# reazon-research/ReazonSpeech

Measured on NVIDIA H100. Metric: RTFx (audio-s/wall-s) FastConformer-RNNT 619M, higher is better.
Workload: dtype bf16

## Files before the change

reazonspeech_b200/csrc/common.cuh:

```cuda
#pragma once
#include <cuda_bf16.h>
#include <cuda_fp16.h>
#include <cuda_runtime.h>
#include <stdint.h>

#include <atomic>

namespace rs {

struct DeviceOnce {
  std::atomic<unsigned long long> done{0};
  bool pending() const { int d = 0; cudaGetDevice(&d); return ((done.load(std::memory_order_acquire) >> (d & 63)) & 1ull) == 0; }
  void set() { int d = 0; cudaGetDevice(&d); done.fetch_or(1ull << (d & 63), std::memory_order_release); }
};

constexpr int kWarp = 32;

__device__ __forceinline__ uint32_t smem_u32(const void* p) {
  return static_cast<uint32_t>(__cvta_generic_to_shared(p));
}
__device__ __forceinline__ int lane_id() { return threadIdx.x & 31; }
__device__ __forceinline__ int warp_id_uniform() { return __shfl_sync(0xffffffffu, threadIdx.x >> 5, 0); }

__device__ __forceinline__ float warp_sum(float v) {
#pragma unroll
  for (int o = 16; o > 0; o >>= 1) v += __shfl_xor_sync(0xffffffffu, v, o);
  return v;
}
__device__ __forceinline__ float warp_max(float v) {
#pragma unroll
  for (int o = 16; o > 0; o >>= 1) v = fmaxf(v, __shfl_xor_sync(0xffffffffu, v, o));
  return v;
}

__device__ __forceinline__ uint32_t pack_bf16x2(float lo, float hi) {
  __nv_bfloat162 t = __floats2bfloat162_rn(lo, hi);
  return *reinterpret_cast<uint32_t*>(&t);
}
__device__ __forceinline__ uint32_t pack_f16x2(float lo, float hi) {
  __half2 t = __floats2half2_rn(lo, hi);
  return *reinterpret_cast<uint32_t*>(&t);
}
__device__ __forceinline__ float2 unpack_bf16x2(uint32_t v) {
  __nv_bfloat162 t = *reinterpret_cast<__nv_bfloat162*>(&v);
  return __bfloat1622float2(t);
}
__device__ __forceinline__ float bf16_lo(uint32_t v) { return __uint_as_float(v << 16); }
__device__ __forceinline__ float bf16_hi(uint32_t v) { return __uint_as_float(v & 0xffff0000u); }

__device__ __forceinline__ void split2(float2 x, uint32_t& hi, uint32_t& lo) {
  constexpr float kMax = 65504.f;
  const __half2 h = __floats2half2_rn(fminf(fmaxf(x.x, -kMax), kMax), fminf(fmaxf(x.y, -kMax), kMax));
  const float2 hf = __half22float2(h);
  const __half2 l = __floats2half2_rn(fminf(fmaxf(x.x - hf.x, -kMax), kMax), fminf(fmaxf(x.y - hf.y, -kMax), kMax));
  hi = *reinterpret_cast<const uint32_t*>(&h);
  lo = *reinterpret_cast<const uint32_t*>(&l);
}

__device__ __forceinline__ uint32_t bf16x2_to_f16x2(uint32_t v) { return pack_f16x2(bf16_lo(v), bf16_hi(v)); }
__device__ __forceinline__ uint4 bf16x8_to_f16x8(uint4 v) {
  return make_uint4(bf16x2_to_f16x2(v.x), bf16x2_to_f16x2(v.y), bf16x2_to_f16x2(v.z), bf16x2_to_f16x2(v.w));
}

__device__ __forceinline__ float sigmoidf_fast(float x) {
  float e, r;
  asm("ex2.approx.ftz.f32 %0, %1;" : "=f"(e) : "f"(x * -1.4426950408889634f));
  asm("rcp.approx.ftz.f32 %0, %1;" : "=f"(r) : "f"(1.0f + e));
  return r;
}
__device__ __forceinline__ float sigmoidf_accurate(float x) { return 1.0f / (1.0f + expf(-x)); }
__device__ __forceinline__ float swishf_fast(float x) { return x * sigmoidf_fast(x); }

__device__ __forceinline__ void mbar_init(uint32_t bar, uint32_t count) {
  asm volatile("mbarrier.init.shared::cta.b64 [%0], %1;" ::"r"(bar), "r"(count));
}
__device__ __forceinline__ void fence_barrier_init() {
  asm volatile("fence.mbarrier_init.release.cluster;" ::: "memory");
}
__device__ __forceinline__ void fence_proxy_async() {
  asm volatile("fence.proxy.async.shared::cta;" ::: "memory");
}
__device__ __forceinline__ void mbar_arrive(uint32_t bar) {
  asm volatile("mbarrier.arrive.shared::cta.b64 _, [%0];" ::"r"(bar) : "memory");
}
__device__ __forceinline__ void mbar_arrive_expect_tx(uint32_t bar, uint32_t bytes) {
  asm volatile("mbarrier.arrive.expect_tx.shared::cta.b64 _, [%0], %1;" ::"r"(bar), "r"(bytes) : "memory");
}
__device__ __forceinline__ bool mbar_try_wait(uint32_t bar, uint32_t parity) {
  uint32_t ok;
  asm volatile(
      "{\n\t.reg .pred p;\n\t"
      "mbarrier.try_wait.parity.shared::cta.b64 p, [%1], %2;\n\t"
      "selp.u32 %0, 1, 0, p;\n\t}"
      : "=r"(ok)
      : "r"(bar), "r"(parity)
      : "memory");
  return ok != 0;
}
__device__ __forceinline__ void mbar_wait(uint32_t bar, uint32_t parity) {
  while (!mbar_try_wait(bar, parity)) {
  }
}

__device__ __forceinline__ void tma_prefetch_desc(const void* desc) {
  asm volatile("prefetch.tensormap [%0];" ::"l"(desc) : "memory");
}
__device__ __forceinline__ void tma_load_2d(uint32_t smem_dst, const void* desc, int c0, int c1, uint32_t bar) {
  asm volatile(
      "cp.async.bulk.tensor.2d.shared::cluster.global.tile.mbarrier::complete_tx::bytes [%0], [%1, {%3, %4}], [%2];"
      ::"r"(smem_dst), "l"(desc), "r"(bar), "r"(c0), "r"(c1)
      : "memory");
}

__device__ __forceinline__ void tma_store_2d(const void* desc, uint32_t smem_src, int c0, int c1) {
  asm volatile("cp.async.bulk.tensor.2d.global.shared::cta.bulk_group [%0, {%2, %3}], [%1];"
               ::"l"(desc), "r"(smem_src), "r"(c0), "r"(c1) : "memory");
}
__device__ __forceinline__ void tma_reduce_add_2d(const void* desc, uint32_t smem_src, int c0, int c1) {
  asm volatile("cp.reduce.async.bulk.tensor.2d.global.shared::cta.add.tile.bulk_group [%0, {%2, %3}], [%1];"
               ::"l"(desc), "r"(smem_src), "r"(c0), "r"(c1) : "memory");
}
__device__ __forceinline__ void bulk_commit() { asm volatile("cp.async.bulk.commit_group;" ::: "memory"); }
template <int N>
__device__ __forceinline__ void bulk_wait_read() { asm volatile("cp.async.bulk.wait_group.read %0;" ::"n"(N) : "memory"); }
template <int N>
__device__ __forceinline__ void bulk_wait() { asm volatile("cp.async.bulk.wait_group %0;" ::"n"(N) : "memory"); }

__device__ __forceinline__ void cp_async16(void* smem, const void* gmem) {
  asm volatile("cp.async.cg.shared.global [%0], [%1], 16;" ::"r"(smem_u32(smem)), "l"(gmem) : "memory");
}
__device__ __forceinline__ void cp_async_wait_all() { asm volatile("cp.async.wait_all;" ::: "memory"); }

__device__ __forceinline__ void stmatrix_x4(uint32_t addr, uint32_t r0, uint32_t r1, uint32_t r2, uint32_t r3) {
  asm volatile("stmatrix.sync.aligned.m8n8.x4.shared.b16 [%0], {%1, %2, %3, %4};"
               ::"r"(addr), "r"(r0), "r"(r1), "r"(r2), "r"(r3) : "memory");
}
__device__ __forceinline__ void stmatrix_x4_trans(uint32_t addr, uint32_t r0, uint32_t r1, uint32_t r2, uint32_t r3) {
  asm volatile("stmatrix.sync.aligned.m8n8.x4.trans.shared.b16 [%0], {%1, %2, %3, %4};"
               ::"r"(addr), "r"(r0), "r"(r1), "r"(r2), "r"(r3) : "memory");
}

template <int N>
__device__ __forceinline__ void setmaxnreg_dec() { asm volatile("setmaxnreg.dec.sync.aligned.u32 %0;" ::"n"(N)); }
template <int N>
__device__ __forceinline__ void setmaxnreg_inc() { asm volatile("setmaxnreg.inc.sync.aligned.u32 %0;" ::"n"(N)); }

__device__ __forceinline__ void wgmma_fence() { asm volatile("wgmma.fence.sync.aligned;" ::: "memory"); }
__device__ __forceinline__ void wgmma_commit() { asm volatile("wgmma.commit_group.sync.aligned;" ::: "memory"); }
template <int N>
__device__ __forceinline__ void wgmma_wait() { asm volatile("wgmma.wait_group.sync.aligned %0;" ::"n"(N) : "memory"); }
__device__ __forceinline__ void named_bar_sync(int id, int threads) { asm volatile("bar.sync %0, %1;" ::"r"(id), "r"(threads) : "memory"); }

__device__ __forceinline__ uint64_t wgmma_desc_k_sw128(uint32_t smem_addr) {
  uint64_t d = 0;
  d |= static_cast<uint64_t>((smem_addr & 0x3ffffu) >> 4);
  d |= static_cast<uint64_t>(1) << 16;
  d |= static_cast<uint64_t>(1024 >> 4) << 32;
  d |= static_cast<uint64_t>(1) << 62;
  return d;
}

__device__ __forceinline__ void wgmma_bf16_ss_n32(float (&d)[16], uint64_t desc_a, uint64_t desc_b, uint32_t accumulate) {
  asm volatile(
      "{\n\t.reg .pred p;\n\t"
      "setp.ne.b32 p, %18, 0;\n\t"
      "wgmma.mma_async.sync.aligned.m64n32k16.f32.bf16.bf16 "
      "{%0, %1, %2, %3, %4, %5, %6, %7, %8, %9, %10, %11, %12, %13, %14, %15}, %16, %17, p, 1, 1, 0, 0;\n\t}"
      :
        "+f"(d[0]), "+f"(d[1]), "+f"(d[2]), "+f"(d[3]), "+f"(d[4]), "+f"(d[5]), "+f"(d[6]), "+f"(d[7]),
        "+f"(d[8]), "+f"(d[9]), "+f"(d[10]), "+f"(d[11]), "+f"(d[12]), "+f"(d[13]), "+f"(d[14]), "+f"(d[15])
      : "l"(desc_a), "l"(desc_b), "r"(accumulate));
}

__device__ __forceinline__ void wgmma_bf16_ss_n64(float (&d)[32], uint64_t desc_a, uint64_t desc_b, uint32_t accumulate) {
  asm volatile(
      "{\n\t.reg .pred p;\n\t"
      "setp.ne.b32 p, %34, 0;\n\t"
      "wgmma.mma_async.sync.aligned.m64n64k16.f32.bf16.bf16 "
      "{%0, %1, %2, %3, %4, %5, %6, %7, %8, %9, %10, %11, %12, %13, %14, %15, %16, %17, %18, %19, %20, %21, %22, %23, %24, %25, %26, %27, %28, %29, %30, %31}, %32, %33, p, 1, 1, 0, 0;\n\t}"
      :
        "+f"(d[0]), "+f"(d[1]), "+f"(d[2]), "+f"(d[3]), "+f"(d[4]), "+f"(d[5]), "+f"(d[6]), "+f"(d[7]),
        "+f"(d[8]), "+f"(d[9]), "+f"(d[10]), "+f"(d[11]), "+f"(d[12]), "+f"(d[13]), "+f"(d[14]), "+f"(d[15]),
        "+f"(d[16]), "+f"(d[17]), "+f"(d[18]), "+f"(d[19]), "+f"(d[20]), "+f"(d[21]), "+f"(d[22]), "+f"(d[23]),
        "+f"(d[24]), "+f"(d[25]), "+f"(d[26]), "+f"(d[27]), "+f"(d[28]), "+f"(d[29]), "+f"(d[30]), "+f"(d[31])
      : "l"(desc_a), "l"(desc_b), "r"(accumulate));
}

__device__ __forceinline__ void wgmma_bf16_ss_n128(float (&d)[64], uint64_t desc_a, uint64_t desc_b, uint32_t accumulate) {
  asm volatile(
      "{\n\t.reg .pred p;\n\t"
      "setp.ne.b32 p, %66, 0;\n\t"
      "wgmma.mma_async.sync.aligned.m64n128k16.f32.bf16.bf16 "
      "{%0, %1, %2, %3, %4, %5, %6, %7, %8, %9, %10, %11, %12, %13, %14, %15, %16, %17, %18, %19, %20, %21, %22, %23, %24, %25, %26, %27, %28, %29, %30, %31, %32, %33, %34, %35, %36, %37, %38, %39, %40, %41, %42, %43, %44, %45, %46, %47, %48, %49, %50, %51, %52, %53, %54, %55, %56, %57, %58, %59, %60, %61, %62, %63}, %64, %65, p, 1, 1, 0, 0;\n\t}"
      :
        "+f"(d[0]), "+f"(d[1]), "+f"(d[2]), "+f"(d[3]), "+f"(d[4]), "+f"(d[5]), "+f"(d[6]), "+f"(d[7]),
        "+f"(d[8]), "+f"(d[9]), "+f"(d[10]), "+f"(d[11]), "+f"(d[12]), "+f"(d[13]), "+f"(d[14]), "+f"(d[15]),
        "+f"(d[16]), "+f"(d[17]), "+f"(d[18]), "+f"(d[19]), "+f"(d[20]), "+f"(d[21]), "+f"(d[22]), "+f"(d[23]),
        "+f"(d[24]), "+f"(d[25]), "+f"(d[26]), "+f"(d[27]), "+f"(d[28]), "+f"(d[29]), "+f"(d[30]), "+f"(d[31]),
        "+f"(d[32]), "+f"(d[33]), "+f"(d[34]), "+f"(d[35]), "+f"(d[36]), "+f"(d[37]), "+f"(d[38]), "+f"(d[39]),
        "+f"(d[40]), "+f"(d[41]), "+f"(d[42]), "+f"(d[43]), "+f"(d[44]), "+f"(d[45]), "+f"(d[46]), "+f"(d[47]),
        "+f"(d[48]), "+f"(d[49]), "+f"(d[50]), "+f"(d[51]), "+f"(d[52]), "+f"(d[53]), "+f"(d[54]), "+f"(d[55]),
        "+f"(d[56]), "+f"(d[57]), "+f"(d[58]), "+f"(d[59]), "+f"(d[60]), "+f"(d[61]), "+f"(d[62]), "+f"(d[63])
      : "l"(desc_a), "l"(desc_b), "r"(accumulate));
}

__device__ __forceinline__ void wgmma_bf16_ss_n256(float (&d)[128], uint64_t desc_a, uint64_t desc_b, uint32_t accumulate) {
  asm volatile(
      "{\n\t.reg .pred p;\n\t"
      "setp.ne.b32 p, %130, 0;\n\t"
      "wgmma.mma_async.sync.aligned.m64n256k16.f32.bf16.bf16 "
      "{%0, %1, %2, %3, %4, %5, %6, %7, %8, %9, %10, %11, %12, %13, %14, %15, %16, %17, %18, %19, %20, %21, %22, %23, %24, %25, %26, %27, %28, %29, %30, %31, "
      "%32, %33, %34, %35, %36, %37, %38, %39, %40, %41, %42, %43, %44, %45, %46, %47, %48, %49, %50, %51, %52, %53, %54, %55, %56, %57, %58, %59, %60, %61, %62, %63, "
      "%64, %65, %66, %67, %68, %69, %70, %71, %72, %73, %74, %75, %76, %77, %78, %79, %80, %81, %82, %83, %84, %85, %86, %87, %88, %89, %90, %91, %92, %93, %94, %95, "
      "%96, %97, %98, %99, %100, %101, %102, %103, %104, %105, %106, %107, %108, %109, %110, %111, %112, %113, %114, %115, %116, %117, %118, %119, %120, %121, %122, %123, %124, %125, %126, %127}, "
      "%128, %129, p, 1, 1, 0, 0;\n\t}"
      :
        "+f"(d[0]), "+f"(d[1]), "+f"(d[2]), "+f"(d[3]), "+f"(d[4]), "+f"(d[5]), "+f"(d[6]), "+f"(d[7]),
        "+f"(d[8]), "+f"(d[9]), "+f"(d[10]), "+f"(d[11]), "+f"(d[12]), "+f"(d[13]), "+f"(d[14]), "+f"(d[15]),
        "+f"(d[16]), "+f"(d[17]), "+f"(d[18]), "+f"(d[19]), "+f"(d[20]), "+f"(d[21]), "+f"(d[22]), "+f"(d[23]),
        "+f"(d[24]), "+f"(d[25]), "+f"(d[26]), "+f"(d[27]), "+f"(d[28]), "+f"(d[29]), "+f"(d[30]), "+f"(d[31]),
        "+f"(d[32]), "+f"(d[33]), "+f"(d[34]), "+f"(d[35]), "+f"(d[36]), "+f"(d[37]), "+f"(d[38]), "+f"(d[39]),
        "+f"(d[40]), "+f"(d[41]), "+f"(d[42]), "+f"(d[43]), "+f"(d[44]), "+f"(d[45]), "+f"(d[46]), "+f"(d[47]),
        "+f"(d[48]), "+f"(d[49]), "+f"(d[50]), "+f"(d[51]), "+f"(d[52]), "+f"(d[53]), "+f"(d[54]), "+f"(d[55]),
        "+f"(d[56]), "+f"(d[57]), "+f"(d[58]), "+f"(d[59]), "+f"(d[60]), "+f"(d[61]), "+f"(d[62]), "+f"(d[63]),
        "+f"(d[64]), "+f"(d[65]), "+f"(d[66]), "+f"(d[67]), "+f"(d[68]), "+f"(d[69]), "+f"(d[70]), "+f"(d[71]),
        "+f"(d[72]), "+f"(d[73]), "+f"(d[74]), "+f"(d[75]), "+f"(d[76]), "+f"(d[77]), "+f"(d[78]), "+f"(d[79]),
        "+f"(d[80]), "+f"(d[81]), "+f"(d[82]), "+f"(d[83]), "+f"(d[84]), "+f"(d[85]), "+f"(d[86]), "+f"(d[87]),
        "+f"(d[88]), "+f"(d[89]), "+f"(d[90]), "+f"(d[91]), "+f"(d[92]), "+f"(d[93]), "+f"(d[94]), "+f"(d[95]),
        "+f"(d[96]), "+f"(d[97]), "+f"(d[98]), "+f"(d[99]), "+f"(d[100]), "+f"(d[101]), "+f"(d[102]), "+f"(d[103]),
        "+f"(d[104]), "+f"(d[105]), "+f"(d[106]), "+f"(d[107]), "+f"(d[108]), "+f"(d[109]), "+f"(d[110]), "+f"(d[111]),
        "+f"(d[112]), "+f"(d[113]), "+f"(d[114]), "+f"(d[115]), "+f"(d[116]), "+f"(d[117]), "+f"(d[118]), "+f"(d[119]),
        "+f"(d[120]), "+f"(d[121]), "+f"(d[122]), "+f"(d[123]), "+f"(d[124]), "+f"(d[125]), "+f"(d[126]), "+f"(d[127])
      : "l"(desc_a), "l"(desc_b), "r"(accumulate));
}

__device__ __forceinline__ void wgmma_f16_ss_n64(float (&d)[32], uint64_t desc_a, uint64_t desc_b, uint32_t accumulate) {
  asm volatile(
      "{\n\t.reg .pred p;\n\t"
      "setp.ne.b32 p, %34, 0;\n\t"
      "wgmma.mma_async.sync.aligned.m64n64k16.f32.f16.f16 "
      "{%0, %1, %2, %3, %4, %5, %6, %7, %8, %9, %10, %11, %12, %13, %14, %15, %16, %17, %18, %19, %20, %21, %22, %23, %24, %25, %26, %27, %28, %29, %30, %31}, %32, %33, p, 1, 1, 0, 0;\n\t}"
      :
        "+f"(d[0]), "+f"(d[1]), "+f"(d[2]), "+f"(d[3]), "+f"(d[4]), "+f"(d[5]), "+f"(d[6]), "+f"(d[7]),
        "+f"(d[8]), "+f"(d[9]), "+f"(d[10]), "+f"(d[11]), "+f"(d[12]), "+f"(d[13]), "+f"(d[14]), "+f"(d[15]),
        "+f"(d[16]), "+f"(d[17]), "+f"(d[18]), "+f"(d[19]), "+f"(d[20]), "+f"(d[21]), "+f"(d[22]), "+f"(d[23]),
        "+f"(d[24]), "+f"(d[25]), "+f"(d[26]), "+f"(d[27]), "+f"(d[28]), "+f"(d[29]), "+f"(d[30]), "+f"(d[31])
      : "l"(desc_a), "l"(desc_b), "r"(accumulate));
}

__device__ __forceinline__ void wgmma_bf16_rs_n128(float (&d)[64], const uint32_t (&a)[4], uint64_t desc_b, uint32_t accumulate) {
  asm volatile(
      "{\n\t.reg .pred p;\n\t"
      "setp.ne.b32 p, %69, 0;\n\t"
      "wgmma.mma_async.sync.aligned.m64n128k16.f32.bf16.bf16 "
      "{%0, %1, %2, %3, %4, %5, %6, %7, %8, %9, %10, %11, %12, %13, %14, %15, %16, %17, %18, %19, %20, %21, %22, %23, %24, %25, %26, %27, %28, %29, %30, %31, %32, %33, %34, %35, %36, %37, %38, %39, %40, %41, %42, %43, %44, %45, %46, %47, %48, %49, %50, %51, %52, %53, %54, %55, %56, %57, %58, %59, %60, %61, %62, %63}, {%64, %65, %66, %67}, %68, p, 1, 1, 0;\n\t}"
      :
        "+f"(d[0]), "+f"(d[1]), "+f"(d[2]), "+f"(d[3]), "+f"(d[4]), "+f"(d[5]), "+f"(d[6]), "+f"(d[7]),
        "+f"(d[8]), "+f"(d[9]), "+f"(d[10]), "+f"(d[11]), "+f"(d[12]), "+f"(d[13]), "+f"(d[14]), "+f"(d[15]),
        "+f"(d[16]), "+f"(d[17]), "+f"(d[18]), "+f"(d[19]), "+f"(d[20]), "+f"(d[21]), "+f"(d[22]), "+f"(d[23]),
        "+f"(d[24]), "+f"(d[25]), "+f"(d[26]), "+f"(d[27]), "+f"(d[28]), "+f"(d[29]), "+f"(d[30]), "+f"(d[31]),
        "+f"(d[32]), "+f"(d[33]), "+f"(d[34]), "+f"(d[35]), "+f"(d[36]), "+f"(d[37]), "+f"(d[38]), "+f"(d[39]),
        "+f"(d[40]), "+f"(d[41]), "+f"(d[42]), "+f"(d[43]), "+f"(d[44]), "+f"(d[45]), "+f"(d[46]), "+f"(d[47]),
        "+f"(d[48]), "+f"(d[49]), "+f"(d[50]), "+f"(d[51]), "+f"(d[52]), "+f"(d[53]), "+f"(d[54]), "+f"(d[55]),
        "+f"(d[56]), "+f"(d[57]), "+f"(d[58]), "+f"(d[59]), "+f"(d[60]), "+f"(d[61]), "+f"(d[62]), "+f"(d[63])
      : "r"(a[0]), "r"(a[1]), "r"(a[2]), "r"(a[3]), "l"(desc_b), "r"(accumulate));
}


__device__ __forceinline__ uint4 ldg_nc_v4(const void* p) {
  uint4 r;
  asm volatile("ld.global.nc.L1::no_allocate.v4.u32 {%0, %1, %2, %3}, [%4];" : "=r"(r.x), "=r"(r.y), "=r"(r.z), "=r"(r.w) : "l"(p));
  return r;
}

}
```

reazonspeech_b200/csrc/gemm_wgmma.cu:

```cuda
#include <cuda.h>
#include <cstdio>
#include <cstdlib>
#include <cstring>

#include "../../include/rs_engine.h"
#include "common.cuh"
#include "kernels.h"

namespace rs {

constexpr int BM = 128;
constexpr int BK = 64;
constexpr int kConsumerWarps = 8;
constexpr int kGemmThreads = 128 + 32 * kConsumerWarps;
constexpr int kABytes = BM * BK * 2;
constexpr int kEpiBufs = 3, kEpiBufBytes = 4096;
constexpr int kBiasBytes = 256 * 4;
constexpr int kProducerRegs = 40, kConsumerRegs = 232;

struct GemmDev {
  const float* bias;
  int M, N, K;
  int epilogue;
  float alpha;
  int split;
};
template <int BN>
struct GemmCfg {
  static constexpr int kBBytes = BN * BK * 2;
  static constexpr int kStageBytes = kABytes + kBBytes;
  static constexpr int kEpiBytes = 2 * (kEpiBufs * kEpiBufBytes + kBiasBytes);
  static constexpr int kFixedBytes = 1024  + 256  + kEpiBytes;
  static constexpr int kStages = (227 * 1024 - kFixedBytes) / kStageBytes;
  static constexpr int kSmemBytes = kStages * kStageBytes + kFixedBytes;
  static_assert(2 * 8 * kStages <= 256, "barrier area");
  static_assert(kStageBytes % 1024 == 0, "epilogue buffers need the 1024 B alignment of the 128 B swizzle");
};

__device__ __forceinline__ uint32_t sw64(int row, int chunk) { return static_cast<uint32_t>(row * 64 + ((chunk ^ ((row >> 1) & 3)) << 4)); }

template <int BN, int EG>
__global__ void __launch_bounds__(kGemmThreads, 1)
gemm_bf16_tn_kernel(const __grid_constant__ CUtensorMap tm_a, const __grid_constant__ CUtensorMap tm_b,
                    const __grid_constant__ CUtensorMap tm_out, const __grid_constant__ CUtensorMap tm_out2, const GemmDev p) {
  using Cfg = GemmCfg<BN>;
  extern __shared__ uint8_t smem_raw[];
  const uint32_t smem_base = (smem_u32(smem_raw) + 1023u) & ~1023u;
  const uint32_t epi_base = smem_base + Cfg::kStages * Cfg::kStageBytes;
  const uint32_t bar_base = epi_base + Cfg::kEpiBytes;
  auto full_bar = [&](int s) { return bar_base + 8u * s; };
  auto empty_bar = [&](int s) { return bar_base + 8u * (Cfg::kStages + s); };
  auto smem_a = [&](int s) { return smem_base + s * Cfg::kStageBytes; };
  auto smem_b = [&](int s) { return smem_base + s * Cfg::kStageBytes + kABytes; };
  auto smem_gen = [&](uint32_t addr) { return smem_raw + (addr - smem_u32(smem_raw)); };

  const int warp = warp_id_uniform();
  const int lane = lane_id();
  const int num_m = (p.M + BM - 1) / BM;
  const int num_n = (p.N + BN - 1) / BN;
  const int num_tiles = num_m * num_n;
  const int num_k = p.K / BK;

  if (threadIdx.x == 0) {
    tma_prefetch_desc(&tm_a);
    tma_prefetch_desc(&tm_b);
    tma_prefetch_desc(&tm_out);
    if constexpr (EG == 1) tma_prefetch_desc(&tm_out2);
    for (int s = 0; s < Cfg::kStages; ++s) { mbar_init(full_bar(s), 1); mbar_init(empty_bar(s), kConsumerWarps); }
    fence_barrier_init();
  }
  __syncthreads();

  if (warp < 4) {
    setmaxnreg_dec<kProducerRegs>();
    if (warp == 0 && lane == 0) {
      int stage = 0; uint32_t phase = 0;
      for (int tile = blockIdx.x; tile < num_tiles; tile += gridDim.x) {
        const int m0 = (tile / num_n) * BM, n0 = (tile % num_n) * BN;
        for (int kb = 0; kb < num_k; ++kb) {
          mbar_wait(empty_bar(stage), phase ^ 1u);
          mbar_arrive_expect_tx(full_bar(stage), Cfg::kStageBytes);
          tma_load_2d(smem_a(stage), &tm_a, kb * BK, m0, full_bar(stage));
          tma_load_2d(smem_b(stage), &tm_b, kb * BK, n0, full_bar(stage));
          if (++stage == Cfg::kStages) { stage = 0; phase ^= 1u; }
        }
      }
    }
  } else {
    setmaxnreg_inc<kConsumerRegs>();
    const int cw = warp - 4;
    const int wg = cw >> 2, wq = cw & 3;
    const int rows0 = wg * 64;
    const int tw = threadIdx.x & 127;
    const uint32_t buf0 = epi_base + wg * kEpiBufs * kEpiBufBytes;
    float* bias_s = reinterpret_cast<float*>(smem_gen(epi_base + 2 * kEpiBufs * kEpiBufBytes + wg * kBiasBytes));
    const int g = lane >> 2, t = lane & 3;
    const int mi = lane >> 3, mr = lane & 7;
    int nbuf = 0;
    auto buf = [&]() { return buf0 + nbuf * kEpiBufBytes; };
    auto flush = [&](const CUtensorMap* map, int c0, int c1, bool reduce) {
      fence_proxy_async();
      if (tw == 0) bulk_wait_read<kEpiBufs - 2>();
      named_bar_sync(1 + wg, 128);
      if (tw == 0) {
        if (reduce) tma_reduce_add_2d(map, buf(), c0, c1);
        else tma_store_2d(map, buf(), c0, c1);
        bulk_commit();
      }
      nbuf = nbuf == kEpiBufs - 1 ? 0 : nbuf + 1;
    };

    int stage = 0; uint32_t phase = 0;
    for (int tile = blockIdx.x; tile < num_tiles; tile += gridDim.x) {
      const int m0 = (tile / num_n) * BM, n0 = (tile % num_n) * BN;
      if (4 * tw < min(BN, p.N - n0)) {
        if (p.bias != nullptr) cp_async16(bias_s + 4 * tw, p.bias + n0 + 4 * tw);
        else *reinterpret_cast<float4*>(bias_s + 4 * tw) = make_float4(0.f, 0.f, 0.f, 0.f);
      }
      float d[BN / 2];
      int prev = -1;
      for (int kb = 0; kb < num_k; ++kb) {
        mbar_wait(full_bar(stage), phase);
        const uint64_t da = wgmma_desc_k_sw128(smem_a(stage) + rows0 * 128);
        const uint64_t db = wgmma_desc_k_sw128(smem_b(stage));
        wgmma_fence();
#pragma unroll
        for (int k = 0; k < BK / 16; ++k) {
          if constexpr (BN == 256) wgmma_bf16_ss_n256(d, da + 2u * k, db + 2u * k, (kb | k) != 0 ? 1u : 0u);
          else wgmma_bf16_ss_n64(d, da + 2u * k, db + 2u * k, (kb | k) != 0 ? 1u : 0u);
        }
        wgmma_commit();
        wgmma_wait<1>();
        if (prev >= 0 && lane == 0) mbar_arrive(empty_bar(prev));
        prev = stage;
        if (++stage == Cfg::kStages) { stage = 0; phase ^= 1u; }
      }
      wgmma_wait<0>();
      if (lane == 0) mbar_arrive(empty_bar(prev));
      cp_async_wait_all();
      named_bar_sync(1 + wg, 128);

      const int row_g = m0 + rows0;
#pragma unroll
      for (int c = 0; c < BN / 32; ++c) {
        const int col0 = n0 + c * 32;
        if (col0 < p.N) {
          float v[4][2][2];
#pragma unroll
          for (int j = 0; j < 4; ++j) {
            const float2 b = *reinterpret_cast<const float2*>(bias_s + 32 * c + 8 * j + 2 * t);
#pragma unroll
            for (int h = 0; h < 2; ++h) { v[j][h][0] = d[16 * c + 4 * j + 2 * h] + b.x; v[j][h][1] = d[16 * c + 4 * j + 2 * h + 1] + b.y; }
          }
          const int epi = EG == 1 ? RS_EPI_QKV_VT : p.epilogue;
          if (EG == 1 && col0 >= p.split) {
#pragma unroll
            for (int q = 0; q < 2; ++q) {
              const int dim = 8 * (2 * q + (mi >> 1)) + mr;
              stmatrix_x4_trans(buf() + dim * 128 + (((2 * wq + (mi & 1)) ^ mr) << 4),
                                pack_bf16x2(v[2 * q][0][0], v[2 * q][0][1]), pack_bf16x2(v[2 * q][1][0], v[2 * q][1][1]),
                                pack_bf16x2(v[2 * q + 1][0][0], v[2 * q + 1][0][1]), pack_bf16x2(v[2 * q + 1][1][0], v[2 * q + 1][1][1]));
            }
            flush(&tm_out2, row_g, col0 - p.split, false);
          } else if (epi == RS_EPI_BIAS_GLU_BF16) {
            uint32_t r[2][2];
#pragma unroll
            for (int j = 0; j < 2; ++j)
#pragma unroll
              for (int h = 0; h < 2; ++h)
                r[j][h] = pack_bf16x2(v[j][h][0] * sigmoidf_fast(v[j + 2][h][0]), v[j][h][1] * sigmoidf_fast(v[j + 2][h][1]));
            stmatrix_x4(buf() + sw64(16 * wq + 8 * (mi & 1) + mr, 2 * (c & 1) + (mi >> 1)), r[0][0], r[0][1], r[1][0], r[1][1]);
            if ((c & 1) || col0 + 32 >= p.N) flush(&tm_out, (col0 & ~63) / 2, row_g, false);
          } else if (epi == RS_EPI_BIAS_F32 || epi == RS_EPI_RESID_F32) {
            const bool swp = (g >> 1) & 1;
#pragma unroll
            for (int s = 0; s < 2; ++s) {
#pragma unroll
              for (int k = 0; k < 2; ++k) {
                const int jl = k ^ static_cast<int>(swp);
#pragma unroll
                for (int h = 0; h < 2; ++h) {
                  const int row = 16 * wq + g + 8 * h;
                  const float a0 = jl ? v[2 * s + 1][h][0] : v[2 * s][h][0], a1 = jl ? v[2 * s + 1][h][1] : v[2 * s][h][1];
                  *reinterpret_cast<float2*>(smem_gen(buf() + sw64(row, 2 * jl + (t >> 1)) + 8 * (t & 1))) =
                      make_float2(a0 * p.alpha, a1 * p.alpha);
                }
              }
              flush(&tm_out, col0 + 16 * s, row_g, epi == RS_EPI_RESID_F32);
            }
          } else {
            uint32_t r[4][2];
#pragma unroll
            for (int j = 0; j < 4; ++j)
#pragma unroll
              for (int h = 0; h < 2; ++h) {
                float x0 = v[j][h][0], x1 = v[j][h][1];
                if (epi == RS_EPI_BIAS_RELU_BF16) { x0 = fmaxf(x0, 0.0f); x1 = fmaxf(x1, 0.0f); }
                else if (epi == RS_EPI_BIAS_SWISH_BF16) { x0 = swishf_fast(x0); x1 = swishf_fast(x1); }
                r[j][h] = epi == RS_EPI_BIAS_F16 ? pack_f16x2(x0, x1) : pack_bf16x2(x0, x1);
              }
#pragma unroll
            for (int q = 0; q < 2; ++q)
              stmatrix_x4(buf() + sw64(16 * wq + 8 * (mi & 1) + mr, 2 * q + (mi >> 1)),
                          r[2 * q][0], r[2 * q][1], r[2 * q + 1][0], r[2 * q + 1][1]);
            flush(&tm_out, col0, row_g, false);
          }
        }
      }
    }
    if (tw == 0) bulk_wait<0>();
  }
}

typedef CUresult (*EncodeTiledFn)(CUtensorMap*, CUtensorMapDataType, cuuint32_t, void*, const cuuint64_t*,
                                  const cuuint64_t*, const cuuint32_t*, const cuuint32_t*, CUtensorMapInterleave,
                                  CUtensorMapSwizzle, CUtensorMapL2promotion, CUtensorMapFloatOOBfill);

static EncodeTiledFn get_encode_fn() {
  static EncodeTiledFn fn = nullptr;
  if (fn == nullptr) {
    void* p = nullptr;
    cudaDriverEntryPointQueryResult qres;
    if (cudaGetDriverEntryPoint("cuTensorMapEncodeTiled", &p, cudaEnableDefault, &qres) == cudaSuccess &&
        qres == cudaDriverEntryPointSuccess)
      fn = reinterpret_cast<EncodeTiledFn>(p);
  }
  return fn;
}

static bool make_tmap_2d(CUtensorMap* m, CUtensorMapDataType dtype, int esize, const void* ptr, uint64_t rows, uint64_t cols,
                         uint64_t ld, uint32_t box_cols, uint32_t box_rows, CUtensorMapSwizzle swizzle, char* err) {
  EncodeTiledFn fn = get_encode_fn();
  if (fn == nullptr) { snprintf(err, 256, "cuTensorMapEncodeTiled entry point unavailable"); return false; }
  cuuint64_t dims[2] = {cols, rows};
  cuuint64_t strides[1] = {ld * esize};
  cuuint32_t box[2] = {box_cols, box_rows};
  cuuint32_t estr[2] = {1, 1};
  CUresult r = fn(m, dtype, 2, const_cast<void*>(ptr), dims, strides, box, estr, CU_TENSOR_MAP_INTERLEAVE_NONE, swizzle,
                  CU_TENSOR_MAP_L2_PROMOTION_L2_256B, CU_TENSOR_MAP_FLOAT_OOB_FILL_NONE);
  if (r != CUDA_SUCCESS) { snprintf(err, 256, "cuTensorMapEncodeTiled failed (%d) rows=%llu cols=%llu", (int)r, (unsigned long long)rows, (unsigned long long)cols); return false; }
  return true;
}

bool make_tmap_bf16(CUtensorMap* m, const void* ptr, uint64_t rows, uint64_t cols, uint64_t ld, uint32_t box_rows, char* err) {
  return make_tmap_2d(m, CU_TENSOR_MAP_DATA_TYPE_BFLOAT16, 2, ptr, rows, cols, ld, BK, box_rows, CU_TENSOR_MAP_SWIZZLE_128B, err);
}

inline int epilogue_group(int epilogue) { return epilogue == RS_EPI_QKV_VT ? 1 : 0; }

template <int BN, int EG>
static cudaError_t launch_bn_eg(const GemmArgs& g, int num_sms, cudaStream_t stream, char* err) {
  using Cfg = GemmCfg<BN>;
  static DeviceOnce attr_once;
  if (attr_once.pending()) {
    cudaError_t e = cudaFuncSetAttribute(gemm_bf16_tn_kernel<BN, EG>, cudaFuncAttributeMaxDynamicSharedMemorySize, Cfg::kSmemBytes);
    if (e != cudaSuccess) { snprintf(err, 256, "cudaFuncSetAttribute(smem=%d): %s", Cfg::kSmemBytes, cudaGetErrorString(e)); return e; }
    attr_once.set();
  }
  CUtensorMap tm_a, tm_b, tm_out, tm_out2;
  if (!make_tmap_bf16(&tm_a, g.a, g.M, g.K, g.K, BM, err)) return cudaErrorInvalidValue;
  if (!make_tmap_bf16(&tm_b, g.w, g.N, g.K, g.K, BN, err)) return cudaErrorInvalidValue;
  const bool f32 = g.epilogue == RS_EPI_RESID_F32 || g.epilogue == RS_EPI_BIAS_F32;
  const int ldo = g.epilogue == RS_EPI_BIAS_GLU_BF16 ? g.N / 2 : g.N;
  const CUtensorMapDataType dt = f32 ? CU_TENSOR_MAP_DATA_TYPE_FLOAT32
                                     : g.epilogue == RS_EPI_BIAS_F16 ? CU_TENSOR_MAP_DATA_TYPE_FLOAT16 : CU_TENSOR_MAP_DATA_TYPE_BFLOAT16;
  if (!make_tmap_2d(&tm_out, dt, f32 ? 4 : 2, g.out, g.M, ldo, ldo, f32 ? 16 : 32, 64, CU_TENSOR_MAP_SWIZZLE_64B, err)) return cudaErrorInvalidValue;
  if (EG == 1 && !make_tmap_2d(&tm_out2, CU_TENSOR_MAP_DATA_TYPE_BFLOAT16, 2, g.out2, g.N - g.split, g.M, g.ld2, 64, 32,
                               CU_TENSOR_MAP_SWIZZLE_128B, err))
    return cudaErrorInvalidValue;
  if (EG == 0) tm_out2 = tm_out;
  GemmDev p{g.bias, g.M, g.N, g.K, g.epilogue, g.alpha, g.split};
  const int tiles = ((g.M + BM - 1) / BM) * ((g.N + BN - 1) / BN);
  const int grid = tiles < num_sms ? tiles : num_sms;
  gemm_bf16_tn_kernel<BN, EG><<<grid, kGemmThreads, Cfg::kSmemBytes, stream>>>(tm_a, tm_b, tm_out, tm_out2, p);
  cudaError_t e = cudaGetLastError();
  if (e != cudaSuccess) snprintf(err, 256, "gemm launch (M=%d N=%d K=%d BN=%d): %s", g.M, g.N, g.K, BN, cudaGetErrorString(e));
  return e;
}

template <int BN>
static cudaError_t launch_bn(const GemmArgs& g, int num_sms, cudaStream_t stream, char* err) {
  switch (epilogue_group(g.epilogue)) {
    case 1: return launch_bn_eg<BN, 1>(g, num_sms, stream, err);
    default: return launch_bn_eg<BN, 0>(g, num_sms, stream, err);
  }
}

cudaError_t launch_gemm(const GemmArgs& g, int num_sms, cudaStream_t stream, char* err) {
  if (g.M <= 0 || g.N <= 0 || g.K <= 0 || g.K % BK != 0 || g.N % 32 != 0) {
    snprintf(err, 256, "gemm shape unsupported: M=%d N=%d K=%d (need K%%64==0, N%%32==0)", g.M, g.N, g.K);
    return cudaErrorInvalidValue;
  }
  if ((reinterpret_cast<uintptr_t>(g.a) | reinterpret_cast<uintptr_t>(g.w) | reinterpret_cast<uintptr_t>(g.out) |
       reinterpret_cast<uintptr_t>(g.bias) | reinterpret_cast<uintptr_t>(g.out2)) & 15u) {
    snprintf(err, 256, "gemm operands, bias and outputs must be 16-byte aligned");
    return cudaErrorInvalidValue;
  }
  if (g.epilogue == RS_EPI_RESID_F32 && g.resid == nullptr) { snprintf(err, 256, "gemm: residual epilogue without resid"); return cudaErrorInvalidValue; }
  if (g.epilogue == RS_EPI_QKV_VT && (g.out2 == nullptr || g.split % 32 || g.ld2 % 8 || g.M % 8 || g.ld2 < g.M)) {
    snprintf(err, 256, "gemm: RS_EPI_QKV_VT needs out2, split %% 32 == 0, ld2 %% 8 == 0, M %% 8 == 0, ld2 >= M");
    return cudaErrorInvalidValue;
  }
  if (g.epilogue == RS_EPI_RESID_F32 && g.resid != g.out) {
    cudaError_t e = cudaMemcpyAsync(g.out, g.resid, static_cast<size_t>(g.M) * g.N * sizeof(float), cudaMemcpyDeviceToDevice, stream);
    if (e != cudaSuccess) { snprintf(err, 256, "gemm: residual copy: %s", cudaGetErrorString(e)); return e; }
  }
  if (g.N % 256 == 0 && ((g.M + BM - 1) / BM) * (g.N / 256) >= num_sms) return launch_bn<256>(g, num_sms, stream, err);
  return launch_bn<64>(g, num_sms, stream, err);
}

}
```

Baseline: 22380.

## Add ping-pong warpgroup schedule with BN=128 tiles for short-K wide GEMMs

Adds a BN=128 GEMM variant in which the two consumer warpgroups each own a whole 128x128 tile from a two-tile unit. Named barriers order their mainloops so one warpgroup's epilogue overlaps the other's tensor-core work. The dispatcher picks this path for large GEMMs with K<=1024 and N>=1024 and keeps BN=256 elsewhere. This targets epilogue stalls on short-K GEMMs, but it adds barrier-ordering complexity and halves the B tile reuse per stage.

```diff
diff --git a/reazonspeech_b200/csrc/common.cuh b/reazonspeech_b200/csrc/common.cuh
--- a/reazonspeech_b200/csrc/common.cuh
+++ b/reazonspeech_b200/csrc/common.cuh
@@ -150,6 +150,7 @@
 template <int N>
 __device__ __forceinline__ void wgmma_wait() { asm volatile("wgmma.wait_group.sync.aligned %0;" ::"n"(N) : "memory"); }
 __device__ __forceinline__ void named_bar_sync(int id, int threads) { asm volatile("bar.sync %0, %1;" ::"r"(id), "r"(threads) : "memory"); }
+__device__ __forceinline__ void named_bar_arrive(int id, int threads) { asm volatile("bar.arrive %0, %1;" ::"r"(id), "r"(threads) : "memory"); }
 
 __device__ __forceinline__ uint64_t wgmma_desc_k_sw128(uint32_t smem_addr) {
   uint64_t d = 0;
diff --git a/reazonspeech_b200/csrc/gemm_wgmma.cu b/reazonspeech_b200/csrc/gemm_wgmma.cu
--- a/reazonspeech_b200/csrc/gemm_wgmma.cu
+++ b/reazonspeech_b200/csrc/gemm_wgmma.cu
@@ -17,6 +17,7 @@
 constexpr int kEpiBufs = 3, kEpiBufBytes = 4096;
 constexpr int kBiasBytes = 256 * 4;
 constexpr int kProducerRegs = 40, kConsumerRegs = 232;
+constexpr int kOrderBar = 3;
 
 struct GemmDev {
   const float* bias;
@@ -27,6 +28,10 @@
 };
 template <int BN>
 struct GemmCfg {
+  static constexpr bool kPingPong = BN == 128;
+  static constexpr int kTilesPerUnit = kPingPong ? 2 : 1;
+  static constexpr int kHalves = kPingPong ? 2 : 1;
+  static constexpr int kStageConsumers = kPingPong ? 4 : 8;
   static constexpr int kBBytes = BN * BK * 2;
   static constexpr int kStageBytes = kABytes + kBBytes;
   static constexpr int kEpiBytes = 2 * (kEpiBufs * kEpiBufBytes + kBiasBytes);
@@ -35,6 +40,7 @@
   static constexpr int kSmemBytes = kStages * kStageBytes + kFixedBytes;
   static_assert(2 * 8 * kStages <= 256, "barrier area");
   static_assert(kStageBytes % 1024 == 0, "epilogue buffers need the 1024 B alignment of the 128 B swizzle");
+  static_assert(kSmemBytes <= 227 * 1024, "shared memory");
 };
 
 __device__ __forceinline__ uint32_t sw64(int row, int chunk) { return static_cast<uint32_t>(row * 64 + ((chunk ^ ((row >> 1) & 3)) << 4)); }
@@ -44,6 +50,7 @@
 gemm_bf16_tn_kernel(const __grid_constant__ CUtensorMap tm_a, const __grid_constant__ CUtensorMap tm_b,
                     const __grid_constant__ CUtensorMap tm_out, const __grid_constant__ CUtensorMap tm_out2, const GemmDev p) {
   using Cfg = GemmCfg<BN>;
+  constexpr bool PP = Cfg::kPingPong;
   extern __shared__ uint8_t smem_raw[];
   const uint32_t smem_base = (smem_u32(smem_raw) + 1023u) & ~1023u;
   const uint32_t epi_base = smem_base + Cfg::kStages * Cfg::kStageBytes;
@@ -58,7 +65,8 @@
   const int lane = lane_id();
   const int num_m = (p.M + BM - 1) / BM;
   const int num_n = (p.N + BN - 1) / BN;
-  const int num_tiles = num_m * num_n;
+  const int units_n = (num_n + Cfg::kTilesPerUnit - 1) / Cfg::kTilesPerUnit;
+  const int num_units = num_m * units_n;
   const int num_k = p.K / BK;
 
   if (threadIdx.x == 0) {
@@ -66,7 +74,7 @@
     tma_prefetch_desc(&tm_b);
     tma_prefetch_desc(&tm_out);
     if constexpr (EG == 1) tma_prefetch_desc(&tm_out2);
-    for (int s = 0; s < Cfg::kStages; ++s) { mbar_init(full_bar(s), 1); mbar_init(empty_bar(s), kConsumerWarps); }
+    for (int s = 0; s < Cfg::kStages; ++s) { mbar_init(full_bar(s), 1); mbar_init(empty_bar(s), Cfg::kStageConsumers); }
     fence_barrier_init();
   }
   __syncthreads();
@@ -75,14 +83,18 @@
     setmaxnreg_dec<kProducerRegs>();
     if (warp == 0 && lane == 0) {
       int stage = 0; uint32_t phase = 0;
-      for (int tile = blockIdx.x; tile < num_tiles; tile += gridDim.x) {
-        const int m0 = (tile / num_n) * BM, n0 = (tile % num_n) * BN;
-        for (int kb = 0; kb < num_k; ++kb) {
-          mbar_wait(empty_bar(stage), phase ^ 1u);
-          mbar_arrive_expect_tx(full_bar(stage), Cfg::kStageBytes);
-          tma_load_2d(smem_a(stage), &tm_a, kb * BK, m0, full_bar(stage));
-          tma_load_2d(smem_b(stage), &tm_b, kb * BK, n0, full_bar(stage));
-          if (++stage == Cfg::kStages) { stage = 0; phase ^= 1u; }
+      for (int unit = blockIdx.x; unit < num_units; unit += gridDim.x) {
+        const int m0 = (unit / units_n) * BM;
+        for (int u = 0; u < Cfg::kTilesPerUnit; ++u) {
+          const int n0 = ((unit % units_n) * Cfg::kTilesPerUnit + u) * BN;
+          if (n0 >= p.N) break;
+          for (int kb = 0; kb < num_k; ++kb) {
+            mbar_wait(empty_bar(stage), phase ^ 1u);
+            mbar_arrive_expect_tx(full_bar(stage), Cfg::kStageBytes);
+            tma_load_2d(smem_a(stage), &tm_a, kb * BK, m0, full_bar(stage));
+            tma_load_2d(smem_b(stage), &tm_b, kb * BK, n0, full_bar(stage));
+            if (++stage == Cfg::kStages) { stage = 0; phase ^= 1u; }
+          }
         }
       }
     }
@@ -90,7 +102,7 @@
     setmaxnreg_inc<kConsumerRegs>();
     const int cw = warp - 4;
     const int wg = cw >> 2, wq = cw & 3;
-    const int rows0 = wg * 64;
+    const int rows0 = PP ? 0 : wg * 64;
     const int tw = threadIdx.x & 127;
     const uint32_t buf0 = epi_base + wg * kEpiBufs * kEpiBufBytes;
     float* bias_s = reinterpret_cast<float*>(smem_gen(epi_base + 2 * kEpiBufs * kEpiBufBytes + wg * kBiasBytes));
@@ -110,39 +122,64 @@
       nbuf = nbuf == kEpiBufs - 1 ? 0 : nbuf + 1;
     };
 
-    int stage = 0; uint32_t phase = 0;
-    for (int tile = blockIdx.x; tile < num_tiles; tile += gridDim.x) {
-      const int m0 = (tile / num_n) * BM, n0 = (tile % num_n) * BN;
-      if (4 * tw < min(BN, p.N - n0)) {
+    uint32_t ring = 0;
+    for (int unit = blockIdx.x; unit < num_units; unit += gridDim.x) {
+      const int m0 = (unit / units_n) * BM;
+      const int nu0 = (unit % units_n) * Cfg::kTilesPerUnit * BN;
+      const int n0 = nu0 + (PP ? wg * BN : 0);
+      const bool has_tile = n0 < p.N;
+      uint32_t stage_it = ring + (PP && wg == 1 ? num_k : 0);
+      ring += num_k * (PP && nu0 + BN >= p.N ? 1 : Cfg::kTilesPerUnit);
+      int stage = static_cast<int>(stage_it % Cfg::kStages);
+      uint32_t phase = (stage_it / Cfg::kStages) & 1u;
+      const bool last_unit = unit + static_cast<int>(gridDim.x) >= num_units;
+
+      if (has_tile && 4 * tw < min(BN, p.N - n0)) {
         if (p.bias != nullptr) cp_async16(bias_s + 4 * tw, p.bias + n0 + 4 * tw);
         else *reinterpret_cast<float4*>(bias_s + 4 * tw) = make_float4(0.f, 0.f, 0.f, 0.f);
       }
-      float d[BN / 2];
-      int prev = -1;
-      for (int kb = 0; kb < num_k; ++kb) {
-        mbar_wait(full_bar(stage), phase);
-        const uint64_t da = wgmma_desc_k_sw128(smem_a(stage) + rows0 * 128);
-        const uint64_t db = wgmma_desc_k_sw128(smem_b(stage));
-        wgmma_fence();
-#pragma unroll
-        for (int k = 0; k < BK / 16; ++k) {
-          if constexpr (BN == 256) wgmma_bf16_ss_n256(d, da + 2u * k, db + 2u * k, (kb | k) != 0 ? 1u : 0u);
-          else wgmma_bf16_ss_n64(d, da + 2u * k, db + 2u * k, (kb | k) != 0 ? 1u : 0u);
+      if (PP && (wg == 1 || unit != static_cast<int>(blockIdx.x))) named_bar_sync(kOrderBar + wg, 256);
+
+      float d[Cfg::kHalves][BN / 2];
+      if (has_tile) {
+        int prev = -1;
+        for (int kb = 0; kb < num_k; ++kb) {
+          mbar_wait(full_bar(stage), phase);
+          const uint64_t da = wgmma_desc_k_sw128(smem_a(stage) + rows0 * 128);
+          const uint64_t db = wgmma_desc_k_sw128(smem_b(stage));
+          wgmma_fence();
+#pragma unroll
+          for (int k = 0; k < BK / 16; ++k) {
+            const uint32_t acc = (kb | k) != 0 ? 1u : 0u;
+            if constexpr (PP) {
+              wgmma_bf16_ss_n128(d[0], da + 2u * k, db + 2u * k, acc);
+              wgmma_bf16_ss_n128(d[1], da + (64u * 128u >> 4) + 2u * k, db + 2u * k, acc);
+            } else if constexpr (BN == 256) {
+              wgmma_bf16_ss_n256(d[0], da + 2u * k, db + 2u * k, acc);
+            } else {
+              wgmma_bf16_ss_n64(d[0], da + 2u * k, db + 2u * k, acc);
+            }
+          }
+          wgmma_commit();
+          wgmma_wait<1>();
+          if (prev >= 0 && lane == 0) mbar_arrive(empty_bar(prev));
+          prev = stage;
+          if (++stage == Cfg::kStages) { stage = 0; phase ^= 1u; }
         }
-        wgmma_commit();
-        wgmma_wait<1>();
-        if (prev >= 0 && lane == 0) mbar_arrive(empty_bar(prev));
-        prev = stage;
-        if (++stage == Cfg::kStages) { stage = 0; phase ^= 1u; }
-      }
-      wgmma_wait<0>();
-      if (lane == 0) mbar_arrive(empty_bar(prev));
-      cp_async_wait_all();
-      named_bar_sync(1 + wg, 128);
-
-      const int row_g = m0 + rows0;
-#pragma unroll
-      for (int c = 0; c < BN / 32; ++c) {
+        if (PP && (wg == 0 || !last_unit)) named_bar_arrive(kOrderBar + (wg ^ 1), 256);
+        wgmma_wait<0>();
+        if (lane == 0) mbar_arrive(empty_bar(prev));
+        cp_async_wait_all();
+        named_bar_sync(1 + wg, 128);
+      } else if (PP && !last_unit) {
+        named_bar_arrive(kOrderBar + 0, 256);
+      }
+      if (!has_tile) continue;
+
+#pragma unroll
+      for (int rc = 0; rc < Cfg::kHalves * (BN / 32); ++rc) {
+        const int r = rc / (BN / 32), c = rc % (BN / 32);
+        const int row_g = m0 + rows0 + 64 * r;
         const int col0 = n0 + c * 32;
         if (col0 < p.N) {
           float v[4][2][2];
@@ -150,7 +187,7 @@
           for (int j = 0; j < 4; ++j) {
             const float2 b = *reinterpret_cast<const float2*>(bias_s + 32 * c + 8 * j + 2 * t);
 #pragma unroll
-            for (int h = 0; h < 2; ++h) { v[j][h][0] = d[16 * c + 4 * j + 2 * h] + b.x; v[j][h][1] = d[16 * c + 4 * j + 2 * h + 1] + b.y; }
+            for (int h = 0; h < 2; ++h) { v[j][h][0] = d[r][16 * c + 4 * j + 2 * h] + b.x; v[j][h][1] = d[r][16 * c + 4 * j + 2 * h + 1] + b.y; }
           }
           const int epi = EG == 1 ? RS_EPI_QKV_VT : p.epilogue;
           if (EG == 1 && col0 >= p.split) {
@@ -163,13 +200,13 @@
             }
             flush(&tm_out2, row_g, col0 - p.split, false);
           } else if (epi == RS_EPI_BIAS_GLU_BF16) {
-            uint32_t r[2][2];
+            uint32_t rr[2][2];
 #pragma unroll
             for (int j = 0; j < 2; ++j)
 #pragma unroll
               for (int h = 0; h < 2; ++h)
-                r[j][h] = pack_bf16x2(v[j][h][0] * sigmoidf_fast(v[j + 2][h][0]), v[j][h][1] * sigmoidf_fast(v[j + 2][h][1]));
-            stmatrix_x4(buf() + sw64(16 * wq + 8 * (mi & 1) + mr, 2 * (c & 1) + (mi >> 1)), r[0][0], r[0][1], r[1][0], r[1][1]);
+                rr[j][h] = pack_bf16x2(v[j][h][0] * sigmoidf_fast(v[j + 2][h][0]), v[j][h][1] * sigmoidf_fast(v[j + 2][h][1]));
+            stmatrix_x4(buf() + sw64(16 * wq + 8 * (mi & 1) + mr, 2 * (c & 1) + (mi >> 1)), rr[0][0], rr[0][1], rr[1][0], rr[1][1]);
             if ((c & 1) || col0 + 32 >= p.N) flush(&tm_out, (col0 & ~63) / 2, row_g, false);
           } else if (epi == RS_EPI_BIAS_F32 || epi == RS_EPI_RESID_F32) {
             const bool swp = (g >> 1) & 1;
@@ -189,7 +226,7 @@
               flush(&tm_out, col0 + 16 * s, row_g, epi == RS_EPI_RESID_F32);
             }
           } else {
-            uint32_t r[4][2];
+            uint32_t rr[4][2];
 #pragma unroll
             for (int j = 0; j < 4; ++j)
 #pragma unroll
@@ -197,12 +234,12 @@
                 float x0 = v[j][h][0], x1 = v[j][h][1];
                 if (epi == RS_EPI_BIAS_RELU_BF16) { x0 = fmaxf(x0, 0.0f); x1 = fmaxf(x1, 0.0f); }
                 else if (epi == RS_EPI_BIAS_SWISH_BF16) { x0 = swishf_fast(x0); x1 = swishf_fast(x1); }
-                r[j][h] = epi == RS_EPI_BIAS_F16 ? pack_f16x2(x0, x1) : pack_bf16x2(x0, x1);
+                rr[j][h] = epi == RS_EPI_BIAS_F16 ? pack_f16x2(x0, x1) : pack_bf16x2(x0, x1);
               }
 #pragma unroll
             for (int q = 0; q < 2; ++q)
               stmatrix_x4(buf() + sw64(16 * wq + 8 * (mi & 1) + mr, 2 * q + (mi >> 1)),
-                          r[2 * q][0], r[2 * q][1], r[2 * q + 1][0], r[2 * q + 1][1]);
+                          rr[2 * q][0], rr[2 * q][1], rr[2 * q + 1][0], rr[2 * q + 1][1]);
             flush(&tm_out, col0, row_g, false);
           }
         }
@@ -270,8 +307,8 @@
     return cudaErrorInvalidValue;
   if (EG == 0) tm_out2 = tm_out;
   GemmDev p{g.bias, g.M, g.N, g.K, g.epilogue, g.alpha, g.split};
-  const int tiles = ((g.M + BM - 1) / BM) * ((g.N + BN - 1) / BN);
-  const int grid = tiles < num_sms ? tiles : num_sms;
+  const int units = ((g.M + BM - 1) / BM) * (((g.N + BN - 1) / BN + Cfg::kTilesPerUnit - 1) / Cfg::kTilesPerUnit);
+  const int grid = units < num_sms ? units : num_sms;
   gemm_bf16_tn_kernel<BN, EG><<<grid, kGemmThreads, Cfg::kSmemBytes, stream>>>(tm_a, tm_b, tm_out, tm_out2, p);
   cudaError_t e = cudaGetLastError();
   if (e != cudaSuccess) snprintf(err, 256, "gemm launch (M=%d N=%d K=%d BN=%d): %s", g.M, g.N, g.K, BN, cudaGetErrorString(e));
@@ -305,7 +342,10 @@
     cudaError_t e = cudaMemcpyAsync(g.out, g.resid, static_cast<size_t>(g.M) * g.N * sizeof(float), cudaMemcpyDeviceToDevice, stream);
     if (e != cudaSuccess) { snprintf(err, 256, "gemm: residual copy: %s", cudaGetErrorString(e)); return e; }
   }
-  if (g.N % 256 == 0 && ((g.M + BM - 1) / BM) * (g.N / 256) >= num_sms) return launch_bn<256>(g, num_sms, stream, err);
+  if (g.N % 256 == 0 && ((g.M + BM - 1) / BM) * (g.N / 256) >= num_sms) {
+    if (g.K <= 1024 && g.N >= 1024) return launch_bn<128>(g, num_sms, stream, err);
+    return launch_bn<256>(g, num_sms, stream, err);
+  }
   return launch_bn<64>(g, num_sms, stream, err);
 }
 
```

Result: faster. 22860, median of 6 (+2.1%).
